# joedane/raytracer-challenge

Measured on AMD Instinct MI355X. Metric: Mrays/sec (primary+shadow), 1920×1080 × 100 spheres; 1/2/4/8 MI355X, higher is better.
Workload: dtype f64

## Files before the change

raytracer-challenge_amd/csrc/rtc_api.cpp:

```cpp
#include <hip/hip_runtime.h>

#include <algorithm>
#include <atomic>
#include <cmath>
#include <cstdlib>
#include <cstring>
#include <new>
#include <type_traits>
#include <vector>

#include "rtc.h"
#include "rtc_ao.h"
#include "rtc_aov.h"
#include "rtc_device.h"
#include "rtc_gather.h"
#include "rtc_internal.h"
#include "rtc_launch_plan.h"
#include "rtc_parity.h"

extern "C" hipError_t rtc_launch_trace(const RenderParams *P, int src, int refl, int refr, uint32_t nblocks,
                                       size_t lds_bytes, hipStream_t stream, hipEvent_t e0, hipEvent_t e1, const DevExtraLights *xl,
                                       const DevLightTable *lt, const DevLens *lens, const DevProjection *proj, int one_sample,
                                       int whole_tiles);
extern "C" hipError_t rtc_launch_prep(const DevIsect *isect, DevPrim *prim, uint32_t n, const double vinv[12],
// ... 437 lines not shown
    HIP_TRY(hipSetDevice(device));
    hipDeviceProp_t prop;
    HIP_TRY(hipGetDeviceProperties(&prop, device));
    if (std::strncmp(prop.gcnArchName, "gfx950", 6) != 0) return RTC_ERR_DEVICE;
    rtc_context *ctx = new (std::nothrow) rtc_context;
    if (!ctx) return RTC_ERR_NOMEM;
    ctx->device = device;
    ctx->stream = static_cast<hipStream_t>(stream);

    if (ctx->d_counters.reserve(CNT_N * CNT_SLOTS) != RTC_OK ||
        hipMemsetAsync(ctx->d_counters.get(), 0, sizeof(unsigned long long) * CNT_N * CNT_SLOTS, ctx->stream) != hipSuccess) {
        rtc_context_destroy(ctx);
        return RTC_ERR_DEVICE;
    }
    if (const char *e = std::getenv("RTC_SRC")) {
        const int v = std::atoi(e);
        if (v >= 0 && v <= 4) ctx->force_src = v;
    }
    if (const char *e = std::getenv("RTC_BINNING")) ctx->binning = std::atoi(e) != 0;
    if (const char *e = std::getenv("RTC_LIGHT_LISTS")) ctx->light_lists = std::atoi(e) != 0;
    if (const char *e = std::getenv("RTC_LIGHT_TABLE")) ctx->light_table = std::atoi(e) != 0;
    if (const char *e = std::getenv("RTC_WORLD_UPDATE")) ctx->world_update = std::atoi(e) != 0;
    if (const char *e = std::getenv("RTC_SKY_ROWS")) ctx->sky_rows = std::atoi(e) != 0;
    if (const char *e = std::getenv("RTC_ONE_SAMPLE")) ctx->one_sample = std::atoi(e) != 0;
    if (const char *e = std::getenv("RTC_WHOLE_TILES")) ctx->whole_tiles = std::atoi(e) != 0;
    if (const char *e = std::getenv("RTC_BIN_SMALL_PIXELS")) ctx->bin_small_pixels = std::strtoull(e, nullptr, 10);
    if (const char *e = std::getenv("RTC_BIN_SMALL_PIXELS_PIPELINED")) ctx->bin_small_pixels_pipelined = std::strtoull(e, nullptr, 10);
    if (const char *e = std::getenv("RTC_TILES_PER_WG")) {
        const int v = std::atoi(e);
        if (v >= 1 && v <= 16) ctx->tiles_per_wg = (uint32_t)v;
    }
    if (const char *e = std::getenv("RTC_TILES_GUIDED")) {
        const long v = std::strtol(e, nullptr, 10);
        if (v >= 0 && v <= 1000) ctx->tiles_guided_tenths = (uint32_t)v;
    }
    if (const char *e = std::getenv("RTC_TILES_SLOTS")) {
        const long v = std::strtol(e, nullptr, 10);
        if (v >= 0 && v <= 1000000) ctx->tiles_slots = (uint32_t)v;
    }
    if (const char *e = std::getenv("RTC_TILES_KMAX")) {
        const long v = std::strtol(e, nullptr, 10);
        if (v >= 1 && v <= 8) ctx->tiles_kmax = (uint32_t)v;
    }
    if (const char *e = std::getenv("RTC_TILE_CAP")) {
        const int v = std::atoi(e);
        if (v >= 16 && v <= 1024) ctx->tile_cap = (uint32_t)v;
// ... 405 lines not shown
    if (w->build_stream) (void)hipStreamDestroy(w->build_stream);
    if (w->pinned) (void)hipHostFree(w->pinned);
    delete w;
}

static bool ready_binset(rtc_context *ctx, rtc_world::BinSet &S, const LaunchPlan &plan, bool sync, hipStream_t stream) {
    if (S.tile_list.capacity() < plan.tiles * RTC_TILE_LIST_CAP) {
        if (sync) (void)hipStreamSynchronize(stream);
        S.tile_cnt.reset();
        S.tile_list.reset();
        if (S.tile_cnt.reserve(plan.tiles_alloc + RTC_BIN_ROW_WORDS, &ctx->render_allocs) != RTC_OK ||
            S.tile_list.reserve(plan.tiles_alloc * RTC_TILE_LIST_CAP, &ctx->render_allocs) != RTC_OK) {
            S.tile_cnt.reset();
            return false;
        }
    }
    if (S.prim.capacity() < plan.prims) {
        if (sync) (void)hipStreamSynchronize(stream);
        if (S.prim.reserve(plan.prims_alloc, &ctx->render_allocs) != RTC_OK) return false;
    }
    return true;
}

static hipError_t bin_tiles(RenderParams &P, const rtc_world::Gen &G, const rtc_world::BinSet &B, const LaunchPlan &plan, bool sky_rows,
                            hipStream_t stream, const hipEvent_t *ev) {
    uint32_t *cnt = B.tile_cnt.get() + RTC_BIN_ROW_WORDS;
    const hipError_t e = rtc_launch_binning(P.views, P.nviews, P.W, P.H, G.n, G.bound_s, G.gbound, G.orig_s,
                                            G.ngroups, cnt, B.tile_list.get(), P.y0 / 8u, P.band_stride, stream, ev ? ev[0] : nullptr,
                                            ev ? ev[1] : nullptr, G.isect_s, G.kind_s, G.n_unb, B.tile_cnt.get(),
                                            G.isect, B.prim.get());
    if (e != hipSuccess) return e;
    P.prim = B.prim.get();
    P.tile_rows = sky_rows ? B.tile_cnt.get() : nullptr;
    P.tile_cnt = cnt;
    P.tile_list = B.tile_list.get();
    P.tiles_x = plan.tiles_x;
    P.tiles_y = plan.tiles_y;
    P.bin_packed = RTC_BIN_PACKED(G.n) ? 1u : 0u;
    P.n_unb = G.n_unb;
    return hipSuccess;
}

struct LaunchRequest {
    const rtc_camera *cams = nullptr;
    uint32_t nviews = 1, view_rows = 0;
    uint32_t mode = 0, y0 = 0, y1 = 0, band_stride = 1, grid_y = 0;
    void *d_rgb = nullptr, *d_rgb8 = nullptr;
    uint32_t flags = 0;
    float gamma = 0.f;
    const rtc_lens *lens = nullptr;
    const rtc_projection *proj = nullptr;
};
static LaunchRequest rows_request(const rtc_camera *cam, uint32_t mode, uint32_t y0, uint32_t y1, void *d_rgb, void *d_rgb8, uint32_t flags) {
    LaunchRequest rq;
    rq.cams = cam; rq.mode = mode; rq.y0 = y0; rq.y1 = y1; rq.grid_y = (y1 - y0 + 7u) / 8u;
    rq.d_rgb = d_rgb; rq.d_rgb8 = d_rgb8; rq.flags = flags;
    return rq;
}
static bool bands_request(const rtc_camera *cam, uint32_t mode, uint32_t first_band, uint32_t band_stride, void *d_rgb, void *d_rgb8,
                          uint32_t flags, LaunchRequest &rq) {
    const uint32_t nbands = (cam->vsize + RTC_BAND_ROWS - 1u) / RTC_BAND_ROWS;
// ... 118 lines not shown
            dproj.row = ctx->d_pano_row.get();
        }
    }
    const bool timed = ctx->time_every != 0 && ctx->launches % ctx->time_every == 0;
    const uint32_t slot = (uint32_t)(ctx->timed % rtc_context::EV_RING);
    if (timed && slot >= ctx->ev_created)
        HIP_TRY(create_events(ctx, std::min<uint32_t>(rtc_context::EV_RING, ctx->ev_created + rtc_context::EV_CHUNK)));
    hipEvent_t *pair = ctx->ev[slot], *pair_bin = ctx->ev_bin[slot];
    const bool piped = ctx->lanes > 1;
    const uint32_t lane = piped && plan.lane_dealt ? (uint32_t)(ctx->lane_next++ % ctx->lanes) : 0u;
    hipStream_t stream = piped ? ctx->lane[lane] : ctx->stream;
    const uint32_t stream_bit = piped ? lane : BIT_STREAM;
    HIP_TRY(order_behind_build(G, stream, stream_bit));
    if (rq.gamma > 0.f) {
        const rtc_status gs = gamma_table(ctx, rq.gamma, stream, piped ? lane : rtc_context::MAX_LANES, &P.gamma);
        if (gs != RTC_OK) return gs;
    }
    rtc_world::BinSet *binset = nullptr;
    int bin_set = -1;
    bool bin_ok = plan.bin != 0u;
    if (bin_ok && piped) {
        rtc_world::BinSet &B = w->bin[lane];
        bin_ok = ready_binset(ctx, B, plan, true, stream);
        if (bin_ok) HIP_TRY(bin_tiles(P, G, B, plan, ctx->sky_rows, stream, timed ? pair_bin : nullptr));
        if (bin_ok) bin_set = (int)lane;
    } else if (bin_ok) {
        if (!ctx->side_stream) HIP_TRY(hipStreamCreateWithFlags(&ctx->side_stream, hipStreamNonBlocking));
        for (uint32_t k = 0; k < 2u && bin_ok; ++k) {
            rtc_world::BinSet &S = w->bin[k];
            if (!S.binned) {
                HIP_TRY(hipEventCreateWithFlags(&S.binned, hipEventDisableTiming));
                HIP_TRY(hipEventCreateWithFlags(&S.traced, hipEventDisableTiming));
            }
            bin_ok = ready_binset(ctx, S, plan, false, stream);
        }
    }
    if (bin_ok && !piped) {
        bin_set = (int)(w->bin_next & 1u);
        rtc_world::BinSet &B = w->bin[w->bin_next++ & 1u];
        HIP_TRY(hipStreamWaitEvent(ctx->side_stream, B.traced, 0));
        HIP_TRY(order_behind_build(G, ctx->side_stream, BIT_SIDE));
        HIP_TRY(bin_tiles(P, G, B, plan, ctx->sky_rows, ctx->side_stream, timed ? pair_bin : nullptr));
        HIP_TRY(hipEventRecord(B.binned, ctx->side_stream));
        HIP_TRY(hipStreamWaitEvent(ctx->stream, B.binned, 0));
        binset = &B;
    }
    if (timed) ctx->bin_timed[slot] = P.tile_cnt != nullptr;
    if (plan.needs_prep) HIP_TRY(rtc_launch_prep(G.isect, w->d_prim.get(), G.n, P.views[0].vinv, stream));
    HIP_TRY(trace_planned(ctx, P, plan, LL, stream, timed ? pair[0] : nullptr, timed ? pair[1] : nullptr, rq.lens ? &dlens : nullptr,
                          rq.proj ? &dproj : nullptr));
    if (binset) HIP_TRY(hipEventRecord(binset->traced, ctx->stream));
    HIP_TRY(record_read(w, G, stream, stream_bit));
    ctx->last = rtc_launch_info{(uint32_t)plan.src, plan.refl, plan.refr, P.tile_cnt ? 1u : 0u, P.light_cnt ? 1u : 0u, lane, plan.block,
                                plan.lds_bytes, plan.reps, plan.chunk_wgs[0] + plan.chunk_wgs[1] + plan.chunk_wgs[2] + plan.chunk_wgs[3],
                                LL.lt ? 1u : 0u, rq.lens ? rq.lens->usteps * rq.lens->vsteps : 0u};
    ctx->last_projection = rq.proj ? rq.proj->kind : 0u;
    ++ctx->launches_total;
    ctx->last_bin = rtc_context::LastBin{};
    if (P.tile_cnt && bin_set >= 0) ctx->last_bin = rtc_context::LastBin{w->serial, (uint32_t)bin_set, rq.nviews, plan.tiles_x, plan.tiles_y};
    ctx->pixels += plan.counted_pixels;
    ++ctx->launches;
    if (timed) ++ctx->timed;
    return RTC_OK;
}

// ... 134 lines not shown
    if (G.light_cap)
        ok = ok && copy(light_cnt, G.lights, sizeof(uint32_t) * LIGHT_CELLS) &&
             copy(light_list, G.lights + LIGHT_CELLS, sizeof(uint32_t) * LIGHT_CELLS * G.light_cap);
    return ok ? RTC_OK : RTC_ERR_DEVICE;
}

extern "C" rtc_status rtc_debug_tile_counts(rtc_context *ctx, const rtc_world *w, uint32_t dims[4], uint32_t *counts, size_t counts_cap,
                                            uint32_t *rows, size_t rows_cap) {
    if (!ctx || !w || !dims || w->ctx != ctx) return RTC_ERR_ARG;
    dims[0] = dims[1] = dims[2] = dims[3] = 0u;
    const rtc_context::LastBin &L = ctx->last_bin;
    if (L.world_serial == 0 || L.world_serial != w->serial) return RTC_OK;
    HIP_TRY(hipSetDevice(ctx->device));
    HIP_TRY(drain_lanes(ctx));
    HIP_TRY(hipStreamSynchronize(ctx->stream));
    if (ctx->side_stream) HIP_TRY(hipStreamSynchronize(ctx->side_stream));
    const rtc_world::BinSet &B = w->bin[L.set];
    const size_t tiles = (size_t)L.nviews * L.tiles_x * L.tiles_y;
    if (!B.tile_cnt.get() || B.tile_cnt.capacity() < RTC_BIN_ROW_WORDS + tiles) return RTC_ERR_ARG;
    if ((counts && counts_cap < tiles) || (rows && rows_cap < 2u * (size_t)L.nviews)) return RTC_ERR_ARG;
    dims[0] = 1u; dims[1] = L.nviews; dims[2] = L.tiles_x; dims[3] = L.tiles_y;
    if (counts) HIP_TRY(hipMemcpy(counts, B.tile_cnt.get() + RTC_BIN_ROW_WORDS, sizeof(uint32_t) * tiles, hipMemcpyDeviceToHost));
    if (rows) HIP_TRY(hipMemcpy(rows, B.tile_cnt.get(), sizeof(uint32_t) * 2u * L.nviews, hipMemcpyDeviceToHost));
    return RTC_OK;
}

rtc_status rtc_stats_reset(rtc_context *ctx) {
    if (!ctx) return RTC_ERR_ARG;
    HIP_TRY(hipSetDevice(ctx->device));
    HIP_TRY(drain_lanes(ctx));
    HIP_TRY(hipMemsetAsync(ctx->d_counters.get(), 0, sizeof(unsigned long long) * CNT_N * CNT_SLOTS, ctx->stream));
    if (ctx->lanes > 1) HIP_TRY(hipStreamSynchronize(ctx->stream));
    ctx->pixels = 0;
    return RTC_OK;
}

rtc_status rtc_context_set_timing(rtc_context *ctx, uint32_t every) {
    if (!ctx) return RTC_ERR_ARG;
    if (every != 0) {
        HIP_TRY(hipSetDevice(ctx->device));
        HIP_TRY(create_events(ctx, std::min<uint32_t>(rtc_context::EV_RING, 64u)));
    }
    ctx->time_every = every;
    ctx->launches = 0;
    ctx->timed = 0;
    return RTC_OK;
// ... 499 lines not shown
```

raytracer-challenge_amd/csrc/rtc_device.h:

```cpp
#ifndef RTC_DEVICE_H
#define RTC_DEVICE_H

#include <stdint.h>

struct DevIsect {
    double m[12];
};

struct DevShade {
    double nt[9];
    double color[3];
    double ambient, diffuse, specular, shininess, reflective, transparency, refractive_index;
    double pat_inv[12];
    double pat_a[3], pat_b[3];
    double plane_n[3];
    uint32_t kind, pattern_kind, world_id, _pad;
};

struct DevPrim {
    double ox, oy, oz;
    double c;
};

struct DevIdEntry {
    uint32_t index, id;
};

struct DevBound {
    double cx, cy, cz, r;
    double k;
    double cn;
};
struct DevPre {
    double cx, cy, cz, R2;
};

struct DevTileBundle {
    float ax, ay, az, cosT, sinT;
    uint32_t off;
};
#define RTC_TILE_LIST_CAP 64u

#define RTC_LIGHT_R 128u
#define RTC_LIGHT_LIST_CAP 128u
#define RTC_LIGHT_LIST_CAP_SMALL 16u


enum { CNT_PRIMARY = 0, CNT_SHADOW = 1, CNT_REFLECT = 2, CNT_REFRACT = 3, CNT_PIXELS = 4, CNT_RESAMPLE = 5, CNT_SKY = 6, CNT_N = 8 };
enum { CNT_SLOTS = 256 };

struct DevCamera {
    double half_width, half_height, pixel_size;
    double vinv[12];
    double origin[3];
    uint32_t origin_ok, _pad;
};
enum { RTC_MAX_VIEWS = 8 };

#ifndef RTC_BLOCK
#define RTC_BLOCK 128
#endif
#ifndef RTC_BLOCK_STACK
#define RTC_BLOCK_STACK 64
#endif
// ... 145 lines not shown
```

raytracer-challenge_amd/csrc/rtc_internal.h:

```cpp
#ifndef RTC_INTERNAL_H
#define RTC_INTERNAL_H

#include <hip/hip_runtime.h>

#include <vector>

#include "rtc.h"
#include "rtc_devmem.h"
#include "rtc_device.h"
#include "rtc_gamma.h"
#include "rtc_world_build.h"

struct rtc_context {
    int device = -1;
    unsigned long long render_allocs = 0;
    unsigned long long pixels = 0;
    hipStream_t stream = nullptr;
    DevBuf<unsigned long long> d_counters;
    static constexpr uint32_t EV_RING = 1024, EV_CHUNK = 16;
    hipEvent_t ev[EV_RING][2] = {};
    hipEvent_t ev_bin[EV_RING][2] = {};
    bool bin_timed[EV_RING] = {};
    uint32_t ev_created = 0;
    uint64_t launches = 0;
// ... 11 lines not shown
    uint32_t tiles_per_wg = 1;
    uint32_t tiles_guided_tenths = 20;
    uint32_t tiles_slots = 0;
    uint32_t tiles_kmax = 8;
    uint32_t tile_cap = 512;
    hipStream_t side_stream = nullptr;
    static constexpr uint32_t MAX_LANES = 4;
    hipStream_t lane[MAX_LANES] = {};
    uint32_t lanes = 1;
    uint64_t lane_next = 0;
    rtc_launch_info last{};
    uint32_t last_projection = 0;
    uint64_t launches_total = 0;
    struct LastBin {
        uint64_t world_serial = 0;
        uint32_t set = 0, nviews = 0, tiles_x = 0, tiles_y = 0;
    } last_bin;
    hipEvent_t fence_ev = nullptr;
    bool light_table = false;
    bool light_lists = true;
    bool world_update = true;
    bool binning = true;
    bool sky_rows = true;
    bool one_sample = true;
    bool whole_tiles = true;
    unsigned long long bin_small_pixels = 6000000ull;
    unsigned long long bin_small_pixels_pipelined = 1500000ull;
    static constexpr uint32_t GAMMA_SLOTS = 16;
    struct GammaSlot {
        bool used = false;
        float gamma = 0.f;
        uint32_t seen = 0;
        hipEvent_t ready = nullptr;
        DevGamma host{};
    };
    DevBuf<DevGamma> d_gamma;
    GammaSlot gamma_slot[GAMMA_SLOTS];
    struct PanoKey {
        uint32_t hsize, vsize;
        double h_span, v_span;
    };
    DevBuf<double> d_pano_col, d_pano_row;
    PanoKey pano_key{};
    bool pano_valid = false;
    unsigned long long pano_uploads = 0;
};
// ... 52 lines not shown
    uint32_t light_cap_alloc = 0;
    unsigned long long allocs = 0;
    mutable bool updated = false;
    hipStream_t build_stream = nullptr;
    unsigned char *pinned = nullptr;
    DevBuf<DevPrim> d_prim;
    struct BinSet {
        DevBuf<uint32_t> tile_cnt, tile_list;
        DevBuf<DevPrim> prim;
        hipEvent_t binned = nullptr;
        hipEvent_t traced = nullptr;
    };
    mutable BinSet bin[rtc_context::MAX_LANES];
    mutable uint32_t bin_next = 0;
    DevBuf<DevTileBundle> d_light_cells;
    bool light_cells_ready = false;
};


extern "C" hipError_t rtc_launch_binning(const DevCamera *views, uint32_t nviews, uint32_t W, uint32_t H, uint32_t n, const DevBound *bound_s,
                                         const DevBound *gbound, const uint32_t *orig_s, uint32_t ngroups, uint32_t *cnt, uint32_t *list,
                                         uint32_t row0, uint32_t row_stride, hipStream_t stream, hipEvent_t e0, hipEvent_t e1,
                                         const DevIsect *isect_s, const uint32_t *kind_s, uint32_t n_unb, uint32_t *rows,
                                         const DevIsect *isect, DevPrim *prim);
enum { RTC_BIN_ROW_WORDS = 2 * RTC_MAX_VIEWS };
extern "C" hipError_t rtc_launch_light_lists(uint32_t n, uint32_t cap, const DevBound *bound, const double light[3], double reach, DevTileBundle *cells,
                                             DevTileBundle *macros, uint32_t *cnt, uint32_t *list, hipStream_t stream);
extern "C" hipError_t rtc_launch_light_lists_built(uint32_t n, uint32_t cap, const DevBound *bound, const double light[3], const DevWorldHeader *hdr,
                                                   const DevTileBundle *cells, const DevTileBundle *macros, uint32_t *cnt, uint32_t *list,
                                                   hipStream_t stream);
extern "C" rtc_status rtc_gamma_build_table(float gamma, DevGamma *g);
extern "C" void rtc_projection_ortho_terms(uint32_t hsize, uint32_t vsize, double width, double out[3]);
extern "C" hipError_t rtc_launch_aov(const AovParams *A, const RenderParams *P, int src, const DevExtraLights *xl, const DevLightTable *lt,
                                     hipStream_t stream);
extern "C" hipError_t rtc_launch_aov_view(const AovViewParams *V, hipStream_t stream);
extern "C" hipError_t rtc_launch_ao(const AoParams *A, const double *dirs, const RenderParams *P, int src, hipStream_t stream);
extern "C" hipError_t rtc_launch_apply_ao(double *rgb, const uint16_t *ao, size_t n, uint32_t n_samples, double strength, hipStream_t stream);
extern "C" hipError_t rtc_launch_gather(const GatherParams *A, const double *dirs, const RenderParams *P, int src, const DevExtraLights *xl,
                                        const DevLightTable *lt, hipStream_t stream);
extern "C" hipError_t rtc_launch_add_scaled(double *rgb, const double *plane, size_t n, double strength, hipStream_t stream);
extern "C" hipError_t rtc_launch_canvas_to_rgba8(const double *rgb, size_t n, const DevGamma *g, unsigned char *out, hipStream_t stream);
struct AverageArgs {
    const double *frames;
    const double *sum_in;
    double *f64_out;
    unsigned char *rgb8, *rgba8;
    const DevGamma *g;
// ... 12 lines not shown
```

raytracer-challenge_amd/csrc/rtc_kernels.hip:

```cpp
#include <hip/hip_runtime.h>
#include <hip/hip_ext.h>

#include <type_traits>

#include "rtc.h"
#include "rtc_ao.h"
#include "rtc_aov.h"
#include "rtc_bands.h"
#include "rtc_device.h"
#include "rtc_gather.h"
#include "rtc_gamma.h"
#include "rtc_parity.h"
#include "rtc_world_build.h"

#define RTC_MAX_STACK 5
#ifndef RTC_WAVES_PER_SIMD
#define RTC_WAVES_PER_SIMD 5
#endif
#ifndef RTC_WAVES_PER_SIMD_STACK
#define RTC_WAVES_PER_SIMD_STACK 4
#endif

#define IS_CULL(S) ((S) == SRC_CULL || (S) == SRC_CULL2)

struct V3 {
    double x, y, z;
};

#define DEVI __device__ __forceinline__

DEVI V3 mk(double x, double y, double z) { V3 v; v.x = x; v.y = y; v.z = z; return v; }
DEVI V3 vadd(V3 a, V3 b) { return mk(a.x + b.x, a.y + b.y, a.z + b.z); }
DEVI V3 vsub(V3 a, V3 b) { return mk(a.x - b.x, a.y - b.y, a.z - b.z); }
DEVI V3 vmul(V3 a, double m) { return mk(a.x * m, a.y * m, a.z * m); }
DEVI V3 vmulv(V3 a, V3 b) { return mk(a.x * b.x, a.y * b.y, a.z * b.z); }
DEVI V3 vneg(V3 a) { return mk(-a.x, -a.y, -a.z); }
DEVI double vdot(V3 a, V3 b) { return a.x * b.x + a.y * b.y + a.z * b.z; }
DEVI V3 vnormalize_plain(V3 a) {
    const double mag = sqrt(a.x * a.x + a.y * a.y + a.z * a.z);
    return mk(a.x / mag, a.y / mag, a.z / mag);
// ... 746 lines not shown

DEVI double reflectance(V3 eyev, V3 normal, double n1, double n2) {
    double cosv = vdot(eyev, normal);
    if (n1 > n2) {
        const double n = n1 / n2;
        const double sin2_t = (n * n) * (1.0 - cosv * cosv);
        if (sin2_t > 1.0) return 1.0;
        cosv = sqrt(1.0 - sin2_t);
    }
    const double q = (n1 - n2) / (n1 + n2);
    const double r0 = q * q;
    const double x = 1.0 - cosv;
    const double x2 = x * x;
    return r0 + (1.0 - r0) * (x * (x2 * x2));
}

typedef const __attribute__((address_space(4))) RenderParams *ParamPtr;
DEVI ParamPtr param_view() {
    unsigned long long a = (unsigned long long)__builtin_amdgcn_kernarg_segment_ptr();
    asm volatile("" : "+s"(a));
    return (ParamPtr)a;
}
#define KP(arg) (*param_view())

template <bool REFR> struct FrameT;
template <> struct FrameT<true> {
    V3 surface;
    V3 a;
    V3 rd;
    double kr, tr, R;
    uint8_t rem;
    uint8_t state;
    uint8_t schlick;
    uint8_t has_refr;
};
template <> struct FrameT<false> {
    V3 surface;
    double kr;
};


template <uint32_t FULL, uint32_t SRC_STRIDE, uint32_t NT>
DEVI void store_rgba(const unsigned char *src8, unsigned char *out8, uint32_t W, uint32_t orow0, uint32_t px0, uint32_t rows,
                     uint32_t cols, uint32_t t) {
    if (cols == FULL && ((size_t)out8 % 4u) == 0) {
        for (uint32_t c = t; c < rows * FULL; c += NT) {
// ... 8 lines not shown
            const unsigned char *q = src8 + r * SRC_STRIDE + x * 3u;
            unsigned char *d = out8 + ((size_t)(orow0 + r) * W + px0 + x) * 4u;
            d[0] = q[0];
            d[1] = q[1];
            d[2] = q[2];
            d[3] = 255u;
        }
    }
}

DEVI double resample_offset(uint32_t W, uint32_t x, uint32_t y, uint32_t draw) {
    unsigned long long z = ((((unsigned long long)y * W + x) << 16) | draw) + 0x9E3779B97F4A7C15ull;
    z = (z ^ (z >> 30)) * 0xBF58476D1CE4E5B9ull;
    z = (z ^ (z >> 27)) * 0x94D049BB133111EBull;
    z ^= z >> 31;
    return (double)(z >> 11) * 0x1p-53;
}

DEVI V3 combine(V3 surface, V3 reflected, V3 refracted, bool schlick, double R) {
    if (schlick) return vadd(surface, vadd(vmul(reflected, R), vmul(refracted, 1.0 - R)));
    return vadd(vadd(surface, reflected), refracted);
}

template <int SRC, bool REFL, bool REFR, bool PROBE, bool RGBA = false, bool ONE = false, bool WHOLE = false, class... XL>
__global__ void __launch_bounds__(RTC_BLOCK_FOR(CULL_LEVEL(SRC), REFL, REFR, PROBE), (REFL ? RTC_WAVES_PER_SIMD_STACK : RTC_WAVES_PER_SIMD))
k_trace(const RenderParams P_arg, const DevIsect *__restrict__ t_isect, const uint32_t *__restrict__ t_kind,
        const DevShade *__restrict__ t_shade, const DevPrim *__restrict__ t_prim, const DevBound *__restrict__ t_bound,
        const DevIsect *__restrict__ t_isect_s, const uint32_t *__restrict__ t_kind_s, const DevBound *__restrict__ t_bound_s,
        const uint32_t *__restrict__ t_orig_s, const DevBound *__restrict__ t_gbound, const DevIdEntry *__restrict__ t_idtab,
        const DevPre *__restrict__ t_pre, const DevPre *__restrict__ t_pre_s, const XL... xl_arg) {
    constexpr bool LENS = has_lens_v<XL...>;
    constexpr bool PROJ = has_projection_v<XL...>;
    constexpr bool ALT = LENS || PROJ;
    constexpr bool MULTI = sizeof...(XL) - (ALT ? 1 : 0) != 0;
    static_assert(!(LENS && PROJ), "a lens or a projection, never both");
    static_assert(sizeof...(XL) <= (ALT ? 2 : 1), "at most one block of further lights, then at most one lens or projection");
    static_assert(!ALT || ((SRC == SRC_SMEM || IS_CULL(SRC)) && !PROBE && !RGBA), "lens and projection launches take SRC_SMEM, SRC_CULL or SRC_CULL2, f64 / RGB output");
    static_assert(!ONE || (IS_CULL(SRC) && !PROBE && !ALT), "the one-sample flavour: pinhole render launches of SRC_CULL and SRC_CULL2");
    static_assert(!WHOLE || (ONE && !RGBA && !MULTI), "the whole-tile flavour: one-sample launches of one light, f64 output");
    constexpr uint32_t BLOCK = RTC_BLOCK_FOR(CULL_LEVEL(SRC), REFL, REFR, PROBE), TILE_W = RTC_TILE_W_FOR(CULL_LEVEL(SRC), REFL, REFR, PROBE);
    extern __shared__ double lds_raw[];
    constexpr bool LDS_STACK = REFL && !REFR;
    constexpr bool WAVE_OUTPUT = REFL;
    constexpr bool SHADOW_LANE_FILTER = SRC == SRC_CULL2 || REFL;
    static_assert(!LDS_STACK || BLOCK == 64, "the tile is staged over the LDS frame stack: one wave per workgroup");
    __shared__ __attribute__((aligned(16))) double stack_lds[LDS_STACK ? RTC_MAX_STACK * 4 * BLOCK : 2];
    __shared__ __attribute__((aligned(16))) double stage_own[(PROBE || LDS_STACK) ? 2 : 8 * TILE_W * 3];
    __shared__ __attribute__((aligned(16))) unsigned char stage_own8[(PROBE || LDS_STACK) ? 16 : 8 * TILE_W * 3];
// ... 46 lines not shown
        by = tbid / P.grid_x;
        bx = tbid - by * P.grid_x;
        px = bx * TILE_W + wave * 8u + (lane & 7u);
        py = P.y0 + by * (WHOLE ? 1u : P.band_stride) * 8u + (lane >> 3);
        in_range = WHOLE || (px < P.W && py < P.y1);
        traced = WHOLE || (in_range && !(P.mode == RTC_MODE_RENDER && (px + 1u >= P.W || py + 1u >= P.H)));
    }

    bool sky_tile = false;
    if constexpr (IS_CULL(SRC) && !PROBE && !ALT) {
        const auto &Pt = KP(P_arg);
        if (Pt.tile_rows != nullptr && (ONE || Pt.samples == 1u)) {
            const uint32_t ity = (Pt.y0 >> 3) + by * (WHOLE ? 1u : Pt.band_stride);
            const uint32_t first = Pt.tile_rows[2u * view], lastinv = Pt.tile_rows[2u * view + 1u];
            sky_tile = ity < first || ity > ~lastinv;
        }
        if (sky_tile) {
            const uint32_t cast = WHOLE ? 64u : popc64(ballot(traced));
            c_primary += cast;
            c_sky += cast;
        }
    }

    bool binned = false;
    uint32_t bin_cnt = 0, bin_ent = 0xffffffffu;
    auto tile_lookup = [&]() {
        const auto &Pt = KP(P_arg);
        if (Pt.tile_cnt != nullptr) {
            const uint32_t wv = (uint32_t)__builtin_amdgcn_readfirstlane((int)wave);
            const uint32_t itx = bx * (TILE_W / 8u) + wv, ity = (Pt.y0 >> 3) + by * (WHOLE ? 1u : Pt.band_stride);
            if (WHOLE || (itx < Pt.tiles_x && ity < Pt.tiles_y)) {
                const size_t tile = (size_t)((WHOLE ? 0u : view * Pt.tiles_y) + ity) * Pt.tiles_x + itx;
                bin_cnt = (uint32_t)__builtin_amdgcn_readfirstlane((int)Pt.tile_cnt[tile]);
                if (lane < bin_cnt) bin_ent = Pt.tile_list[tile * RTC_TILE_LIST_CAP + lane];
                binned = bin_cnt <= RTC_TILE_LIST_CAP;
            }
        }
    };

    const bool aa = !ONE && !ALT && !probe && P.samples != 1u;
    uint32_t nsamples = aa ? 4u : 1u;
    uint32_t lens_u = 0u, lens_v = 0u;
    V3 lens_sum = mk(0., 0., 0.);
    if constexpr (LENS) {
        const DevLens &LZ = last_of(xl_arg...);
        nsamples = LZ.usteps * LZ.vsteps;
    }
    bool lane_resample = false;
    double *aa_store = reinterpret_cast<double *>(reinterpret_cast<char *>(lds_raw) + P.aa_lds_off) + threadIdx.x * 15u;
    V3 result = mk(0., 0., 0.);

    typedef FrameT<REFR> Frame;
    Frame stack[(REFL && !LDS_STACK) ? RTC_MAX_STACK : 1];
    double *lstk = stack_lds + threadIdx.x;

    for (uint32_t s = sky_tile ? nsamples : 0u; s < nsamples; ++s) {
        V3 ro, rd;
// ... 90 lines not shown
            if constexpr (IS_CULL(SRC)) {
                if (ballot(tracing) != 0ull && !use_bins) {
                    if (shared_origin && first) B = make_bundle<true, false>(tracing, cam_origin, ro, rd, 0.);
                    else B = make_bundle<false, false>(tracing, cam_origin, ro, rd, 0.);
                }
            }
            if (!IS_CULL(SRC) && !ALT && shared_origin && first) {
                for_each_object<SRC>(P, T, L, tracing, B, [&](int j, auto m, uint32_t kind, auto pr) {
                    if (tracing) closest_prim(kind, m, pr, rd, j, best, hidx, hroot);
                    return true;
                });
            } else if (IS_CULL(SRC) && REFL && !(shared_origin && first)) {
                for_each_object<SRC, true>(P, T, L, tracing, B, ClosestHit{tracing, ro, rd, best, hidx, hroot}, ro, rd);
            } else if (IS_CULL(SRC) && !PROBE && use_bins) {
                const auto &Pb = KP(P_arg);
                const DevPrim *__restrict__ vprim = WHOLE ? T.prim : T.prim + (size_t)view * Pb.n;
                auto binned_test = [&](uint32_t kind, const double *m, uint32_t j) {
                    closest_prim(kind, m, reinterpret_cast<const double *>(vprim + j), rd, (int)j, best, hidx, hroot);
                };
                for (uint32_t k = 0; k < Pb.n_unb; ++k) {
                    const uint32_t jo = T.orig_s[k];
                    if (tracing) binned_test(T.kind_s[k], T.isect_s[k].m, jo);
                }
                if (Pb.bin_packed) {
                    uint32_t ent = lane < bin_cnt ? bin_ent : 0xffffffffu;
                    for (;;) {
                        const uint32_t e = ~wave_max_u32(~ent);
                        if (e == 0xffffffffu) break;
                        const float kmin = __builtin_bit_cast(float, e & 0xffff0000u);
                        if (ballot(tracing && !(best < (double)kmin)) == 0ull) break;
                        if (ent == e) ent = 0xffffffffu;
                        const uint32_t j = e & 0xffffu;
                        if (tracing) binned_test(T.kind[j], T.isect[j].m, j);
                    }
                } else {
                    uint32_t my_j = 0u;
                    float my_key = 0.f;
                    if (lane < bin_cnt) {
                        my_j = bin_ent;
                        my_key = bound_key(cam_origin, T.bound[my_j]);
                    }
                    unsigned long long lmask = bin_cnt >= 64u ? ~0ull : ((1ull << bin_cnt) - 1ull);
                    while (lmask) {
                        float kmin;
                        const int sel = take_min_key(lmask, my_key, kmin);
                        if (ballot(tracing && !(best < (double)kmin)) == 0ull) break;
                        const uint32_t j = (uint32_t)__builtin_amdgcn_readlane((int)my_j, sel);
                        if (tracing) binned_test(T.kind[j], T.isect[j].m, j);
                    }
                }
            } else if (SRC == SRC_CULL2 && !PROBE && shared_origin && first) {
                for_each_object<SRC, false>(P, T, L, tracing, B, ClosestHit{tracing, ro, rd, best, hidx, hroot}, ro, rd, [&](float key) { return ballot(tracing && !(best < (double)key)) == 0ull; });
            } else {
                for_each_object<SRC>(P, T, L, tracing, B, ClosestHit{tracing, ro, rd, best, hidx, hroot}, ro, rd);
            }
            const bool hit = tracing && hidx >= 0;
            const auto &Ph = KP(P_arg);
            const V3 lightp = mk(Ph.light_pos[0], Ph.light_pos[1], Ph.light_pos[2]);

            V3 point = mk(0, 0, 0), eyev = mk(0, 0, 0), normal = mk(0, 0, 0), over = mk(0, 0, 0), under = mk(0, 0, 0),
// ... 657 lines not shown
}

DEVI uint32_t bin_entry(const BinParams &Q, V3 o, const DevBound &b, uint32_t j) {
    if (!Q.packed) return j;
    return (__builtin_bit_cast(uint32_t, bound_key(o, b)) & 0xffff0000u) | j;
}

DEVI bool cone_misses_plane(const double *m, V3 o, const DevTileBundle &t) {
#pragma clang fp contract(fast)
    if (t.off != 0u) return false;
    const double oy = m[4] * o.x + m[5] * o.y + m[6] * o.z + m[7];
    if (!(fabs(oy) >= 0x1p-500) || !(fabs(oy) < __builtin_inf())) return false;
    const double s = oy > 0. ? 1. : -1.;
    const double rx = m[4], ry = m[5], rz = m[6];
    const double rr = rx * rx + ry * ry + rz * rz;
    if (!(rr > 0x1p-900) || !(rr < 0x1p900)) return false;
    const double ra = s * (rx * (double)t.ax + ry * (double)t.ay + rz * (double)t.az);
    if (!(ra > 0.)) return false;
    const double perp = __builtin_sqrt(fmax(0., rr - ra * ra) * 1.00001 + 1e-10 * rr);
    const double lower = ra * (double)t.cosT * 0.99999 - perp * (double)t.sinT;
    return lower > 1e-4 * __builtin_sqrt(rr);
}

__global__ void __launch_bounds__(64) k_bin_tiles(const BinParams Q, const DevBound *__restrict__ bound_s, const DevBound *__restrict__ gbound,
                                                   const uint32_t *__restrict__ orig_s, uint32_t ngroups, uint32_t *__restrict__ cnt,
                                                   uint32_t *__restrict__ list, const DevIsect *__restrict__ isect_s,
                                                   const uint32_t *__restrict__ kind_s, uint32_t n_unb, uint32_t *__restrict__ rows,
                                                   const DevIsect *__restrict__ isect, DevPrim *__restrict__ prim) {
    const uint32_t macros = Q.macros_x * Q.macros_y;
    const uint32_t view = blockIdx.x / macros, m = blockIdx.x % macros, lane = threadIdx.x;
    if (prim != nullptr) {
        const V3 cam = xpoint(Q.views[view].vinv, mk(0., 0., 0.));
        for (uint32_t j = m * 64u + lane; j < Q.n; j += macros * 64u) prim[(size_t)view * Q.n + j] = prim_of(isect[j].m, cam);
    }
    const uint32_t mx = m % Q.macros_x, my = m / Q.macros_x;
    const uint32_t tx = mx * 8u + (lane & 7u), ty = my * 8u + (lane >> 3);
    const bool mine = tx < Q.tiles_x && ty < Q.tiles_y && ty >= Q.row0 && (ty - Q.row0) % Q.row_stride == 0u;
    if (ballot(mine) == 0ull) return;
    const DevCamera &C = Q.views[view];
    V3 o = xpoint(C.vinv, mk(0., 0., 0.));
    o = mk(uniform_f64(o.x), uniform_f64(o.y), uniform_f64(o.z));
    const Bundle MB = bundle_of(cell_cone(Q, view, mx * 64u, my * 64u, 64u), o);
    const DevTileBundle tcone = cell_cone(Q, view, min(tx, Q.tiles_x - 1u) * 8u, min(ty, Q.tiles_y - 1u) * 8u, 8u);
    const Bundle TB = bundle_of(tcone, o);
    const size_t tile = (size_t)(view * Q.tiles_y + min(ty, Q.tiles_y - 1u)) * Q.tiles_x + min(tx, Q.tiles_x - 1u);
    uint32_t *my_list = list + tile * RTC_TILE_LIST_CAP;
    uint32_t my_cnt = 0;
    bool clear_of_planes = n_unb <= 4u;
    for (uint32_t k = 0; k < n_unb && n_unb <= 4u; ++k)
        clear_of_planes = clear_of_planes && (kind_s[k] == RTC_PLANE) && cone_misses_plane(isect_s[k].m, o, tcone);
    for (uint32_t gbase = 0; gbase < ngroups; gbase += 64u) {
// ... 9 lines not shown
        uint32_t o_next = 0u;
        if (gmask) fetch(gbase + (uint32_t)__builtin_ctzll(gmask), b_next, o_next);
        while (gmask) {
            const uint32_t gsel = gbase + (uint32_t)__builtin_ctzll(gmask);
            gmask &= gmask - 1ull;
            const DevBound b = b_next;
            const uint32_t orig = o_next;
            if (gmask) fetch(gbase + (uint32_t)__builtin_ctzll(gmask), b_next, o_next);
            const uint32_t k = gsel * 64u + lane;
            bool to = false;
            uint32_t entry = 0u;
            if (k < Q.n) {
                to = b.r < __builtin_inf() && bundle_touches(MB, b);
                if (to) entry = bin_entry(Q, o, b, orig);
            }
            unsigned long long omask = ballot(to);
            while (omask) {
                const uint32_t l = (uint32_t)__builtin_ctzll(omask);
                omask &= omask - 1ull;
                const DevBound bj = DevBound{lane_f64(b.cx, l), lane_f64(b.cy, l), lane_f64(b.cz, l), lane_f64(b.r, l), lane_f64(b.k, l), lane_f64(b.cn, l)};
                const uint32_t ej = (uint32_t)__builtin_amdgcn_readlane((int)entry, (int)l);
                if (mine && bundle_touches(TB, bj)) {
                    if (my_cnt < RTC_TILE_LIST_CAP) my_list[my_cnt] = ej;
                    ++my_cnt;
                }
            }
        }
    }
    if (mine) cnt[tile] = my_cnt;
    const bool nonempty = mine && !(my_cnt == 0u && clear_of_planes);
    const uint32_t rmin = ~wave_max_u32(nonempty ? ~ty : 0u), rmaxinv = ~wave_max_u32(nonempty ? ty : 0u);
    const bool any_nonempty = ballot(nonempty) != 0ull;
    if (lane == 0u && any_nonempty) {
        volatile uint32_t *rw = rows + 2u * view;
        if (rmin < rw[0]) atomicMin(rows + 2u * view, rmin);
        if (rmaxinv < rw[1]) atomicMin(rows + 2u * view + 1u, rmaxinv);
    }
}

extern "C" hipError_t rtc_launch_binning(const DevCamera *views, uint32_t nviews, uint32_t W, uint32_t H, uint32_t n, const DevBound *bound_s,
                                         const DevBound *gbound, const uint32_t *orig_s, uint32_t ngroups, uint32_t *cnt, uint32_t *list,
                                         uint32_t row0, uint32_t row_stride, hipStream_t stream, hipEvent_t e0, hipEvent_t e1,
                                         const DevIsect *isect_s, const uint32_t *kind_s, uint32_t n_unb, uint32_t *rows,
                                         const DevIsect *isect, DevPrim *prim) {
    if (n == 0) return hipSuccess;
    if (hipMemsetAsync(rows, 0xff, sizeof(uint32_t) * 2u * RTC_MAX_VIEWS, stream) != hipSuccess) return hipGetLastError();
    BinParams Q;
    Q.row0 = row0; Q.row_stride = row_stride ? row_stride : 1u;
    for (uint32_t v = 0; v < nviews; ++v) Q.views[v] = views[v];
    for (uint32_t v = nviews; v < RTC_MAX_VIEWS; ++v) Q.views[v] = views[0];
    Q.nviews = nviews; Q.W = W; Q.H = H; Q.n = n;
    Q.packed = RTC_BIN_PACKED(n) ? 1u : 0u;
    Q.tiles_x = (W + 7u) / 8u; Q.tiles_y = (H + 7u) / 8u;
    Q.macros_x = (Q.tiles_x + 7u) / 8u; Q.macros_y = (Q.tiles_y + 7u) / 8u;
    hipExtLaunchKernelGGL(k_bin_tiles, dim3(nviews * Q.macros_x * Q.macros_y), dim3(64), 0, stream, e0, e1, 0, Q, bound_s, gbound, orig_s, ngroups, cnt, list,
                          isect_s, kind_s, n_unb, rows, isect, prim);
    return hipGetLastError();
}

DEVI void light_dir(uint32_t face, float u, float v, float &x, float &y, float &z) {
    const float s = (face & 1u) ? -1.f : 1.f;
    const uint32_t a = face >> 1;
    float c[3];
    c[a] = s; c[(a + 1u) % 3u] = u; c[(a + 2u) % 3u] = v;
    const float il = __builtin_amdgcn_rsqf(c[0] * c[0] + c[1] * c[1] + c[2] * c[2]);
    x = c[0] * il; y = c[1] * il; z = c[2] * il;
}
__global__ void __launch_bounds__(256) k_light_cells(DevTileBundle *__restrict__ cells, DevTileBundle *__restrict__ macros, uint32_t *__restrict__ cnt) {
#pragma clang fp contract(fast)
    constexpr uint32_t R = RTC_LIGHT_R, M = RTC_LIGHT_R / 8u;
    uint32_t i = blockIdx.x * 256u + threadIdx.x;
    uint32_t g, span;
    DevTileBundle *out;
    if (i < 6u * R * R) { g = R; span = 1u; out = cells; cnt[i] = 0u; }
    else if ((i -= 6u * R * R) < 6u * M * M) { g = M; span = 8u; out = macros; }
    else return;
    const uint32_t face = i / (g * g), ix = (i % g) * span, iy = ((i / g) % g) * span;
    const float u0 = (float)ix * (2.f / R) - 1.f, u1 = (float)(ix + span) * (2.f / R) - 1.f;
    const float v0 = (float)iy * (2.f / R) - 1.f, v1 = (float)(iy + span) * (2.f / R) - 1.f;
// ... 673 lines not shown
```

Measured before the change: 76910.

## Pre-sort tile bin lists by depth key and walk them with scalar loads

The binning kernel gains a SORT variant that ranks each tile's packed entries (key in high bits, index in low bits) in LDS for lists up to 16 entries, so each tile list is stored in ascending near-bound order. For cull-mode, non-reflective traces, the trace kernel then reads the tile list through constant (scalar) address-space loads and walks entries sequentially, stopping early once no lane's best hit can be beaten. This replaces the per-iteration wave-max selection loop with a sorted scalar walk. The cost is extra sorting work and LDS in binning, plus a separate launch-bounds knob for whole-tile kernels. A debug API for dumping tile lists is also added.

```diff
diff --git a/raytracer-challenge_amd/csrc/rtc_api.cpp b/raytracer-challenge_amd/csrc/rtc_api.cpp
--- a/raytracer-challenge_amd/csrc/rtc_api.cpp
+++ b/raytracer-challenge_amd/csrc/rtc_api.cpp
@@ -483,6 +483,7 @@
     if (const char *e = std::getenv("RTC_LIGHT_TABLE")) ctx->light_table = std::atoi(e) != 0;
     if (const char *e = std::getenv("RTC_WORLD_UPDATE")) ctx->world_update = std::atoi(e) != 0;
     if (const char *e = std::getenv("RTC_SKY_ROWS")) ctx->sky_rows = std::atoi(e) != 0;
+    if (const char *e = std::getenv("RTC_BIN_SORT")) ctx->bin_sort = std::atoi(e) != 0;
     if (const char *e = std::getenv("RTC_ONE_SAMPLE")) ctx->one_sample = std::atoi(e) != 0;
     if (const char *e = std::getenv("RTC_WHOLE_TILES")) ctx->whole_tiles = std::atoi(e) != 0;
     if (const char *e = std::getenv("RTC_BIN_SMALL_PIXELS")) ctx->bin_small_pixels = std::strtoull(e, nullptr, 10);
@@ -934,13 +935,15 @@
     return true;
 }
 
-static hipError_t bin_tiles(RenderParams &P, const rtc_world::Gen &G, const rtc_world::BinSet &B, const LaunchPlan &plan, bool sky_rows,
+static hipError_t bin_tiles(const rtc_context *ctx, RenderParams &P, const rtc_world::Gen &G, const rtc_world::BinSet &B, const LaunchPlan &plan,
                             hipStream_t stream, const hipEvent_t *ev) {
+    const bool sort = ctx->bin_sort && plan.src == SRC_CULL && !plan.refl;
+    const bool sky_rows = ctx->sky_rows;
     uint32_t *cnt = B.tile_cnt.get() + RTC_BIN_ROW_WORDS;
     const hipError_t e = rtc_launch_binning(P.views, P.nviews, P.W, P.H, G.n, G.bound_s, G.gbound, G.orig_s,
                                             G.ngroups, cnt, B.tile_list.get(), P.y0 / 8u, P.band_stride, stream, ev ? ev[0] : nullptr,
                                             ev ? ev[1] : nullptr, G.isect_s, G.kind_s, G.n_unb, B.tile_cnt.get(),
-                                            G.isect, B.prim.get());
+                                            G.isect, B.prim.get(), sort ? 1u : 0u);
     if (e != hipSuccess) return e;
     P.prim = B.prim.get();
     P.tile_rows = sky_rows ? B.tile_cnt.get() : nullptr;
@@ -948,7 +951,7 @@
     P.tile_list = B.tile_list.get();
     P.tiles_x = plan.tiles_x;
     P.tiles_y = plan.tiles_y;
-    P.bin_packed = RTC_BIN_PACKED(G.n) ? 1u : 0u;
+    P.bin_packed = RTC_BIN_PACKED(G.n) ? (sort ? 2u : 1u) : 0u;
     P.n_unb = G.n_unb;
     return hipSuccess;
 }
@@ -1113,7 +1116,7 @@
     if (bin_ok && piped) {
         rtc_world::BinSet &B = w->bin[lane];
         bin_ok = ready_binset(ctx, B, plan, true, stream);
-        if (bin_ok) HIP_TRY(bin_tiles(P, G, B, plan, ctx->sky_rows, stream, timed ? pair_bin : nullptr));
+        if (bin_ok) HIP_TRY(bin_tiles(ctx, P, G, B, plan, stream, timed ? pair_bin : nullptr));
         if (bin_ok) bin_set = (int)lane;
     } else if (bin_ok) {
         if (!ctx->side_stream) HIP_TRY(hipStreamCreateWithFlags(&ctx->side_stream, hipStreamNonBlocking));
@@ -1131,7 +1134,7 @@
         rtc_world::BinSet &B = w->bin[w->bin_next++ & 1u];
         HIP_TRY(hipStreamWaitEvent(ctx->side_stream, B.traced, 0));
         HIP_TRY(order_behind_build(G, ctx->side_stream, BIT_SIDE));
-        HIP_TRY(bin_tiles(P, G, B, plan, ctx->sky_rows, ctx->side_stream, timed ? pair_bin : nullptr));
+        HIP_TRY(bin_tiles(ctx, P, G, B, plan, ctx->side_stream, timed ? pair_bin : nullptr));
         HIP_TRY(hipEventRecord(B.binned, ctx->side_stream));
         HIP_TRY(hipStreamWaitEvent(ctx->stream, B.binned, 0));
         binset = &B;
@@ -1312,6 +1315,23 @@
     dims[0] = 1u; dims[1] = L.nviews; dims[2] = L.tiles_x; dims[3] = L.tiles_y;
     if (counts) HIP_TRY(hipMemcpy(counts, B.tile_cnt.get() + RTC_BIN_ROW_WORDS, sizeof(uint32_t) * tiles, hipMemcpyDeviceToHost));
     if (rows) HIP_TRY(hipMemcpy(rows, B.tile_cnt.get(), sizeof(uint32_t) * 2u * L.nviews, hipMemcpyDeviceToHost));
+    return RTC_OK;
+}
+
+extern "C" rtc_status rtc_debug_tile_lists(rtc_context *ctx, const rtc_world *w, uint32_t dims[4], uint32_t *lists, size_t lists_cap) {
+    if (!ctx || !w || !dims || !lists || w->ctx != ctx) return RTC_ERR_ARG;
+    dims[0] = dims[1] = dims[2] = dims[3] = 0u;
+    const rtc_context::LastBin &L = ctx->last_bin;
+    if (L.world_serial == 0 || L.world_serial != w->serial) return RTC_OK;
+    HIP_TRY(hipSetDevice(ctx->device));
+    HIP_TRY(drain_lanes(ctx));
+    HIP_TRY(hipStreamSynchronize(ctx->stream));
+    if (ctx->side_stream) HIP_TRY(hipStreamSynchronize(ctx->side_stream));
+    const rtc_world::BinSet &B = w->bin[L.set];
+    const size_t words = (size_t)L.nviews * L.tiles_x * L.tiles_y * RTC_TILE_LIST_CAP;
+    if (!B.tile_list.get() || B.tile_list.capacity() < words || lists_cap < words) return RTC_ERR_ARG;
+    dims[0] = 1u; dims[1] = L.nviews; dims[2] = L.tiles_x; dims[3] = L.tiles_y;
+    HIP_TRY(hipMemcpy(lists, B.tile_list.get(), sizeof(uint32_t) * words, hipMemcpyDeviceToHost));
     return RTC_OK;
 }
 
diff --git a/raytracer-challenge_amd/csrc/rtc_device.h b/raytracer-challenge_amd/csrc/rtc_device.h
--- a/raytracer-challenge_amd/csrc/rtc_device.h
+++ b/raytracer-challenge_amd/csrc/rtc_device.h
@@ -40,6 +40,7 @@
     uint32_t off;
 };
 #define RTC_TILE_LIST_CAP 64u
+#define RTC_TILE_SORT_CAP 16u
 
 #define RTC_LIGHT_R 128u
 #define RTC_LIGHT_LIST_CAP 128u
diff --git a/raytracer-challenge_amd/csrc/rtc_internal.h b/raytracer-challenge_amd/csrc/rtc_internal.h
--- a/raytracer-challenge_amd/csrc/rtc_internal.h
+++ b/raytracer-challenge_amd/csrc/rtc_internal.h
@@ -57,6 +57,7 @@
     bool world_update = true;
     bool binning = true;
     bool sky_rows = true;
+    bool bin_sort = true;
     bool one_sample = true;
     bool whole_tiles = true;
     unsigned long long bin_small_pixels = 6000000ull;
@@ -155,7 +156,7 @@
                                          const DevBound *gbound, const uint32_t *orig_s, uint32_t ngroups, uint32_t *cnt, uint32_t *list,
                                          uint32_t row0, uint32_t row_stride, hipStream_t stream, hipEvent_t e0, hipEvent_t e1,
                                          const DevIsect *isect_s, const uint32_t *kind_s, uint32_t n_unb, uint32_t *rows,
-                                         const DevIsect *isect, DevPrim *prim);
+                                         const DevIsect *isect, DevPrim *prim, uint32_t sort);
 enum { RTC_BIN_ROW_WORDS = 2 * RTC_MAX_VIEWS };
 extern "C" hipError_t rtc_launch_light_lists(uint32_t n, uint32_t cap, const DevBound *bound, const double light[3], double reach, DevTileBundle *cells,
                                              DevTileBundle *macros, uint32_t *cnt, uint32_t *list, hipStream_t stream);
diff --git a/raytracer-challenge_amd/csrc/rtc_kernels.hip b/raytracer-challenge_amd/csrc/rtc_kernels.hip
--- a/raytracer-challenge_amd/csrc/rtc_kernels.hip
+++ b/raytracer-challenge_amd/csrc/rtc_kernels.hip
@@ -14,8 +14,15 @@
 #include "rtc_world_build.h"
 
 #define RTC_MAX_STACK 5
-#ifndef RTC_WAVES_PER_SIMD
+#ifdef RTC_WAVES_PER_SIMD
+#ifndef RTC_WAVES_PER_SIMD_WHOLE
+#define RTC_WAVES_PER_SIMD_WHOLE RTC_WAVES_PER_SIMD
+#endif
+#else
 #define RTC_WAVES_PER_SIMD 5
+#endif
+#ifndef RTC_WAVES_PER_SIMD_WHOLE
+#define RTC_WAVES_PER_SIMD_WHOLE 5
 #endif
 #ifndef RTC_WAVES_PER_SIMD_STACK
 #define RTC_WAVES_PER_SIMD_STACK 4
@@ -808,6 +815,16 @@
     return (ParamPtr)a;
 }
 #define KP(arg) (*param_view())
+typedef const __attribute__((address_space(4))) uint32_t *ConstWords;
+DEVI ConstWords const_words(const uint32_t *p) { return (ConstWords)(unsigned long long)p; }
+#ifndef RTC_SCALAR_TILE_WALK
+#define RTC_SCALAR_TILE_WALK 1
+#endif
+constexpr bool trace_scalar_walk(int src, bool refl, bool one, int lights) {
+    if (RTC_SCALAR_TILE_WALK == 0 || src != SRC_CULL || refl) return false;
+    if (!one && lights != 0) return false;
+    return true;
+}
 
 template <bool REFR> struct FrameT;
 template <> struct FrameT<true> {
@@ -862,8 +879,12 @@
     return vadd(vadd(surface, reflected), refracted);
 }
 
+constexpr int trace_waves_per_simd(int src, bool refl, bool one, bool whole) {
+    if (refl) return RTC_WAVES_PER_SIMD_STACK;
+    return (src == SRC_CULL && one && whole) ? RTC_WAVES_PER_SIMD_WHOLE : RTC_WAVES_PER_SIMD;
+}
 template <int SRC, bool REFL, bool REFR, bool PROBE, bool RGBA = false, bool ONE = false, bool WHOLE = false, class... XL>
-__global__ void __launch_bounds__(RTC_BLOCK_FOR(CULL_LEVEL(SRC), REFL, REFR, PROBE), (REFL ? RTC_WAVES_PER_SIMD_STACK : RTC_WAVES_PER_SIMD))
+__global__ void __launch_bounds__(RTC_BLOCK_FOR(CULL_LEVEL(SRC), REFL, REFR, PROBE), trace_waves_per_simd(SRC, REFL, ONE, WHOLE))
 k_trace(const RenderParams P_arg, const DevIsect *__restrict__ t_isect, const uint32_t *__restrict__ t_kind,
         const DevShade *__restrict__ t_shade, const DevPrim *__restrict__ t_prim, const DevBound *__restrict__ t_bound,
         const DevIsect *__restrict__ t_isect_s, const uint32_t *__restrict__ t_kind_s, const DevBound *__restrict__ t_bound_s,
@@ -956,8 +977,12 @@
         }
     }
 
+    constexpr int LIGHTS = (false || ... || __is_same(XL, DevExtraLights)) ? 1 : (false || ... || __is_same(XL, DevLightTable)) ? 2 : 0;
+    constexpr bool SCALAR_WALK = IS_CULL(SRC) && !PROBE && !ALT && trace_scalar_walk(SRC, REFL, ONE, LIGHTS);
     bool binned = false;
     uint32_t bin_cnt = 0, bin_ent = 0xffffffffu;
+    ConstWords bin_list = nullptr;
+    uint32_t bin_head = 0;
     auto tile_lookup = [&]() {
         const auto &Pt = KP(P_arg);
         if (Pt.tile_cnt != nullptr) {
@@ -965,8 +990,14 @@
             const uint32_t itx = bx * (TILE_W / 8u) + wv, ity = (Pt.y0 >> 3) + by * (WHOLE ? 1u : Pt.band_stride);
             if (WHOLE || (itx < Pt.tiles_x && ity < Pt.tiles_y)) {
                 const size_t tile = (size_t)((WHOLE ? 0u : view * Pt.tiles_y) + ity) * Pt.tiles_x + itx;
-                bin_cnt = (uint32_t)__builtin_amdgcn_readfirstlane((int)Pt.tile_cnt[tile]);
-                if (lane < bin_cnt) bin_ent = Pt.tile_list[tile * RTC_TILE_LIST_CAP + lane];
+                if constexpr (SCALAR_WALK) {
+                    bin_list = const_words(Pt.tile_list) + tile * RTC_TILE_LIST_CAP;
+                    bin_cnt = const_words(Pt.tile_cnt)[tile];
+                    bin_head = bin_list[0];
+                } else {
+                    bin_cnt = (uint32_t)__builtin_amdgcn_readfirstlane((int)Pt.tile_cnt[tile]);
+                    if (lane < bin_cnt) bin_ent = Pt.tile_list[tile * RTC_TILE_LIST_CAP + lane];
+                }
                 binned = bin_cnt <= RTC_TILE_LIST_CAP;
             }
         }
@@ -1103,7 +1134,20 @@
                     const uint32_t jo = T.orig_s[k];
                     if (tracing) binned_test(T.kind_s[k], T.isect_s[k].m, jo);
                 }
-                if (Pb.bin_packed) {
+                if (SCALAR_WALK && Pb.bin_packed == 2u && bin_cnt <= RTC_TILE_SORT_CAP) {
+                    uint32_t e_next = bin_head;
+                    for (uint32_t k = 0; k < bin_cnt; ++k) {
+                        const uint32_t e = e_next;
+                        e_next = bin_list[k + 1u];
+                        const float kmin = __builtin_bit_cast(float, e & 0xffff0000u);
+                        if (ballot(tracing && !(best < (double)kmin)) == 0ull) break;
+                        const uint32_t j = e & 0xffffu;
+                        if (tracing) binned_test(T.kind[j], T.isect[j].m, j);
+                    }
+                } else if (Pb.bin_packed) {
+                    if constexpr (SCALAR_WALK) {
+                        if (lane < bin_cnt) bin_ent = ((const uint32_t *)(unsigned long long)bin_list)[lane];
+                    }
                     uint32_t ent = lane < bin_cnt ? bin_ent : 0xffffffffu;
                     for (;;) {
                         const uint32_t e = ~wave_max_u32(~ent);
@@ -1117,6 +1161,9 @@
                 } else {
                     uint32_t my_j = 0u;
                     float my_key = 0.f;
+                    if constexpr (SCALAR_WALK) {
+                        if (lane < bin_cnt) bin_ent = ((const uint32_t *)(unsigned long long)bin_list)[lane];
+                    }
                     if (lane < bin_cnt) {
                         my_j = bin_ent;
                         my_key = bound_key(cam_origin, T.bound[my_j]);
@@ -1820,11 +1867,13 @@
     return lower > 1e-4 * __builtin_sqrt(rr);
 }
 
+template <bool SORT>
 __global__ void __launch_bounds__(64) k_bin_tiles(const BinParams Q, const DevBound *__restrict__ bound_s, const DevBound *__restrict__ gbound,
                                                    const uint32_t *__restrict__ orig_s, uint32_t ngroups, uint32_t *__restrict__ cnt,
                                                    uint32_t *__restrict__ list, const DevIsect *__restrict__ isect_s,
                                                    const uint32_t *__restrict__ kind_s, uint32_t n_unb, uint32_t *__restrict__ rows,
                                                    const DevIsect *__restrict__ isect, DevPrim *__restrict__ prim) {
+    __shared__ uint32_t ents[SORT ? 64u * (RTC_TILE_SORT_CAP + 1u) : 1u];
     const uint32_t macros = Q.macros_x * Q.macros_y;
     const uint32_t view = blockIdx.x / macros, m = blockIdx.x % macros, lane = threadIdx.x;
     if (prim != nullptr) {
@@ -1880,8 +1929,29 @@
                 const uint32_t ej = (uint32_t)__builtin_amdgcn_readlane((int)entry, (int)l);
                 if (mine && bundle_touches(TB, bj)) {
                     if (my_cnt < RTC_TILE_LIST_CAP) my_list[my_cnt] = ej;
+                    if constexpr (SORT) {
+                        if (my_cnt < RTC_TILE_SORT_CAP) ents[lane * (RTC_TILE_SORT_CAP + 1u) + my_cnt] = ej;
+                    }
                     ++my_cnt;
                 }
+            }
+        }
+    }
+    if constexpr (SORT) {
+        const uint32_t c = my_cnt <= RTC_TILE_SORT_CAP ? my_cnt : 0u;
+        const uint32_t cmax = wave_max_u32(c);
+        if (cmax >= 2u) {
+            const uint32_t *const row = ents + lane * (RTC_TILE_SORT_CAP + 1u);
+            uint32_t v[RTC_TILE_SORT_CAP];
+#pragma unroll
+            for (uint32_t k = 0; k < RTC_TILE_SORT_CAP; ++k) v[k] = k < c ? row[k] : 0xffffffffu;
+#pragma unroll
+            for (uint32_t e = 0; e < RTC_TILE_SORT_CAP; ++e) {
+                if (e >= cmax) break;
+                uint32_t rank = 0u;
+#pragma unroll
+                for (uint32_t k = 0; k < RTC_TILE_SORT_CAP; ++k) rank += v[k] < v[e] ? 1u : 0u;
+                if (e < c) my_list[rank] = v[e];
             }
         }
     }
@@ -1900,7 +1970,7 @@
                                          const DevBound *gbound, const uint32_t *orig_s, uint32_t ngroups, uint32_t *cnt, uint32_t *list,
                                          uint32_t row0, uint32_t row_stride, hipStream_t stream, hipEvent_t e0, hipEvent_t e1,
                                          const DevIsect *isect_s, const uint32_t *kind_s, uint32_t n_unb, uint32_t *rows,
-                                         const DevIsect *isect, DevPrim *prim) {
+                                         const DevIsect *isect, DevPrim *prim, uint32_t sort) {
     if (n == 0) return hipSuccess;
     if (hipMemsetAsync(rows, 0xff, sizeof(uint32_t) * 2u * RTC_MAX_VIEWS, stream) != hipSuccess) return hipGetLastError();
     BinParams Q;
@@ -1911,8 +1981,13 @@
     Q.packed = RTC_BIN_PACKED(n) ? 1u : 0u;
     Q.tiles_x = (W + 7u) / 8u; Q.tiles_y = (H + 7u) / 8u;
     Q.macros_x = (Q.tiles_x + 7u) / 8u; Q.macros_y = (Q.tiles_y + 7u) / 8u;
-    hipExtLaunchKernelGGL(k_bin_tiles, dim3(nviews * Q.macros_x * Q.macros_y), dim3(64), 0, stream, e0, e1, 0, Q, bound_s, gbound, orig_s, ngroups, cnt, list,
-                          isect_s, kind_s, n_unb, rows, isect, prim);
+    const dim3 grid(nviews * Q.macros_x * Q.macros_y);
+    if (sort != 0u && Q.packed != 0u)
+        hipExtLaunchKernelGGL(k_bin_tiles<true>, grid, dim3(64), 0, stream, e0, e1, 0, Q, bound_s, gbound, orig_s, ngroups, cnt, list, isect_s, kind_s, n_unb,
+                              rows, isect, prim);
+    else
+        hipExtLaunchKernelGGL(k_bin_tiles<false>, grid, dim3(64), 0, stream, e0, e1, 0, Q, bound_s, gbound, orig_s, ngroups, cnt, list, isect_s, kind_s, n_unb,
+                              rows, isect, prim);
     return hipGetLastError();
 }
 
```

New measurement: 78530, median of 6. +2.1%, better.
